# imironhead/ml_super_resolution

Measured on AMD Instinct MI355X. Metric: VDSR-20 training patches/sec (41x41, batch 256 per GPU); fwd HR megapixels/sec alongside, higher is better.
Workload: dtype f32; 1 GPU; BASELINE configs[2]: VDSR 20-layer 3x3x64 residual, RGB, batch 256x41x41 per GPU, fwd+bwd+TF-Adam, random-init weights; global_batch=256, patch=41, parallelism=dp1

## Files before the change

include/srx.h:

```cpp
#ifndef SRX_H_
#define SRX_H_

#include <stddef.h>
#include <stdint.h>

#ifdef __cplusplus
extern "C" {
#endif

typedef void* srx_stream_t;

typedef enum {
    SRX_OK = 0,
    SRX_ERR_BAD_ARG = -1,
    SRX_ERR_UNSUPPORTED = -2,
    SRX_ERR_WORKSPACE = -3,
    SRX_ERR_LAUNCH = -4,
    SRX_ERR_ALIGN = -5
} srx_status;

typedef enum { SRX_PAD_SAME = 0, SRX_PAD_VALID = 1 } srx_pad_mode;

typedef enum {
    SRX_ACT_NONE = 0,
    SRX_ACT_RELU = 1,
    SRX_ACT_TANH = 2,
    SRX_ACT_LRELU = 3,
    SRX_ACT_SIGMOID = 4
} srx_act;

typedef enum { SRX_OP_FWD = 0, SRX_OP_BWD_DATA = 1, SRX_OP_BWD_FILTER = 2 } srx_conv_op;

typedef enum { SRX_PRECISION_FP32 = 0, SRX_PRECISION_BF16X3 = 1 } srx_precision;

typedef struct {
    int32_t N, H, W, Cin, Cout, KH, KW;
    int32_t stride;
    int32_t pad_mode;
    int32_t act;
    int32_t post_add_relu;
    int32_t precision;
    int32_t subpixel_r;
} srx_conv_desc;

const char* srx_version(void);
const char* srx_last_error(void);

int srx_set_conv_path(int pipelined);

int srx_set_wgrad_path(int path);

int srx_conv2d_precision_supported(const srx_conv_desc* d, int op);

size_t srx_conv2d_workspace_bytes(const srx_conv_desc* d, int op);

int srx_conv2d_fwd(const srx_conv_desc* d, const float* x, const float* w, const float* bias,
                   const float* skip, float* y, void* ws, size_t ws_bytes, srx_stream_t stream);

int srx_conv2d_bwd_data(const srx_conv_desc* d, const float* dpre, const float* w,
                        const float* x_in, int in_act, float* dx_out, void* ws, size_t ws_bytes,
                        srx_stream_t stream);

int srx_conv2d_bwd_data_acc(const srx_conv_desc* d, const float* dpre, const float* w, const float* dx_acc,
                            float* dx_out, void* ws, size_t ws_bytes, srx_stream_t stream);

int srx_conv2d_bwd_filter(const srx_conv_desc* d, const float* x, const float* dpre, float* dw,
                          float* dbias, const float* w_for_decay, float wd_scale, void* ws,
                          size_t ws_bytes, srx_stream_t stream);

int srx_conv2d_bwd_filter_partials(const srx_conv_desc* d, const float* x, const float* dpre, void* ws,
                                   size_t ws_bytes, int* n_partials, srx_stream_t stream);
int srx_conv2d_bwd_filter_reduce(const srx_conv_desc* d, const void* ws, int n_partials, float* dw,
                                 float* dbias, const float* w_for_decay, float wd_scale,
                                 srx_stream_t stream);

int srx_act_bwd(const float* dy, const float* y, float* dpre, size_t numel, int act,
                srx_stream_t stream);

int srx_depth_to_space(const float* in, float* out, int N, int H, int W, int C, int r,
                       srx_stream_t stream);

int srx_stream_copy(const void* in, void* out, size_t bytes, srx_stream_t stream);

// ... 137 lines not shown
```

ml_super_resolution_amd/_lib.py:

```python
import ctypes
import os

_HERE = os.path.dirname(os.path.abspath(__file__))
LIB_PATH = os.path.join(_HERE, 'libsrx.so')

SRX_OK = 0
PAD_SAME, PAD_VALID = 0, 1
ACT_NONE, ACT_RELU, ACT_TANH, ACT_LRELU, ACT_SIGMOID = 0, 1, 2, 3, 4
OP_FWD, OP_BWD_DATA, OP_BWD_FILTER = 0, 1, 2
PRECISION_FP32, PRECISION_BF16X3 = 0, 1
PRECISION_BY_NAME = {'highest': PRECISION_FP32, 'high': PRECISION_BF16X3}

ACT_BY_NAME = {None: ACT_NONE, 'none': ACT_NONE, 'relu': ACT_RELU, 'tanh': ACT_TANH,
               'lrelu': ACT_LRELU, 'leaky_relu': ACT_LRELU, 'sigmoid': ACT_SIGMOID}
PAD_BY_NAME = {'same': PAD_SAME, 'valid': PAD_VALID}

EXPORTS = [
    'srx_version', 'srx_last_error', 'srx_set_conv_path', 'srx_set_wgrad_path', 'srx_conv2d_precision_supported', 'srx_conv2d_workspace_bytes', 'srx_conv2d_fwd',
    'srx_conv2d_bwd_data', 'srx_conv2d_bwd_filter', 'srx_conv2d_bwd_filter_partials', 'srx_conv2d_bwd_filter_reduce', 'srx_act_bwd', 'srx_depth_to_space',
    'srx_space_to_depth', 'srx_stream_copy', 'srx_mse_fwd_bwd', 'srx_l2_loss', 'srx_reduce_scratch_bytes',
    'srx_adam_tf_step', 'srx_adam_tf_step_dev', 'srx_momentum_clip_step', 'srx_rownorm_loss_fwd_bwd', 'srx_psnr', 'srx_ssim', 'srx_ssim_scratch_bytes', 'srx_saturate_u8', 'srx_affine', 'srx_u8_to_unit_float', 'srx_gaussian_blur', 'srx_resize_bilinear',
    'srx_upsample_nearest', 'srx_upsample_nearest_bwd', 'srx_add_relu_grad',
    'srx_conv2d_bwd_data_acc', 'srx_conv3x3_blocked', 'srx_conv3x3_blocked_bwd_filter_workspace_bytes', 'srx_conv3x3_blocked_bwd_filter',
    'srx_espcn_forward', 'srx_espcn_forward_keep', 'srx_debug_poison_lds', 'srx_srcnn_forward', 'srx_maxpool2x2', 'srx_maxpool2x2_bwd', 'srx_maxpool2x2_bwd_masked', 'srx_subsample2', 'srx_subsample2_bwd',
    'srx_channel_blocks_to_nhwc', 'srx_nhwc_to_channel_blocks', 'srx_channel_normalize', 'srx_channel_normalize_bwd',
    'srx_extract_patches16', 'srx_texture_gram', 'srx_texture_gram_bwd', 'srx_pil_resample_ksize', 'srx_pil_resample_coeffs', 'srx_resample_u8', 'srx_u8_to_pm1', 'srx_log_loss', 'srx_vgg_preprocess', 'srx_add_scaled', 'srx_resize_bicubic_tf', 'srx_column_sums', 'srx_gemm_workspace_bytes', 'srx_gemm',
]


class SrxError(RuntimeError):
    pass


class ConvDesc(ctypes.Structure):
    _fields_ = [(n, ctypes.c_int32) for n in
                ('N', 'H', 'W', 'Cin', 'Cout', 'KH', 'KW', 'stride', 'pad_mode', 'act',
                 'post_add_relu', 'precision', 'subpixel_r')]


class GemmDesc(ctypes.Structure):
    _fields_ = ([(n, ctypes.c_int32) for n in ('M', 'N', 'K', 'batch')] +
                [(n, ctypes.c_int64) for n in ('a_row_stride', 'a_col_stride', 'a_batch_stride', 'b_row_stride',
                                               'b_col_stride', 'b_batch_stride', 'c_row_stride', 'c_col_stride',
                                               'c_batch_stride')] +
                [('alpha', ctypes.c_float), ('act', ctypes.c_int32), ('accumulate', ctypes.c_int32)])


_lib = None


def lib():
    global _lib
    if _lib is not None:
        return _lib
    if not os.path.exists(LIB_PATH):
        raise SrxError('libsrx.so not found at %s -- build it with `make -C %s` (or '
                       '__graft_entry__.build()); there is no CPU fallback' %
                       (LIB_PATH, os.path.join(_HERE, 'csrc')))
    import torch
    L = ctypes.CDLL(LIB_PATH)
    vp, sz, i, f = ctypes.c_void_p, ctypes.c_size_t, ctypes.c_int, ctypes.c_float
    dp = ctypes.POINTER(ConvDesc)
    L.srx_version.restype = ctypes.c_char_p
    L.srx_last_error.restype = ctypes.c_char_p
    L.srx_set_conv_path.argtypes = [i]
    L.srx_set_wgrad_path.argtypes = [i]
    L.srx_conv2d_precision_supported.argtypes = [dp, i]
    L.srx_conv2d_workspace_bytes.argtypes = [dp, i]
    L.srx_conv2d_workspace_bytes.restype = sz
    L.srx_reduce_scratch_bytes.restype = sz
    L.srx_conv2d_fwd.argtypes = [dp, vp, vp, vp, vp, vp, vp, sz, vp]
    L.srx_conv2d_bwd_data.argtypes = [dp, vp, vp, vp, i, vp, vp, sz, vp]
    L.srx_conv2d_bwd_filter.argtypes = [dp, vp, vp, vp, vp, vp, f, vp, sz, vp]
    L.srx_conv2d_bwd_filter_partials.argtypes = [dp, vp, vp, vp, sz, ctypes.POINTER(ctypes.c_int), vp]
    L.srx_conv2d_bwd_filter_reduce.argtypes = [dp, vp, i, vp, vp, vp, f, vp]
    L.srx_act_bwd.argtypes = [vp, vp, vp, sz, i, vp]
    L.srx_depth_to_space.argtypes = [vp, vp, i, i, i, i, i, vp]
    L.srx_space_to_depth.argtypes = [vp, vp, i, i, i, i, i, vp]
    L.srx_stream_copy.argtypes = [vp, vp, sz, vp]
    L.srx_mse_fwd_bwd.argtypes = [vp, vp, sz, f, vp, i, vp, vp, vp]
    L.srx_l2_loss.argtypes = [vp, vp, sz, f, vp, i, vp, vp]
    L.srx_adam_tf_step.argtypes = [vp, vp, vp, vp, sz, f, f, f, f, ctypes.c_int64, f, vp]
    L.srx_adam_tf_step_dev.argtypes = [vp, vp, vp, vp, sz, vp, f, f, f, f, vp]
    L.srx_momentum_clip_step.argtypes = [vp, vp, vp, sz, f, f, f, f, vp]
    L.srx_rownorm_loss_fwd_bwd.argtypes = [vp, vp, sz, sz, vp, vp, vp, vp]
    L.srx_psnr.argtypes = [vp, vp, vp, i, sz, f, vp]
    L.srx_ssim.argtypes = [vp, vp, vp, i, i, i, i, f, vp, vp]
    L.srx_ssim_scratch_bytes.argtypes = [i]
    L.srx_ssim_scratch_bytes.restype = sz
    L.srx_saturate_u8.argtypes = [vp, vp, sz, vp]
    L.srx_affine.argtypes = [vp, vp, sz, f, f, vp]
    L.srx_u8_to_unit_float.argtypes = [vp, vp, sz, vp]
    L.srx_gaussian_blur.argtypes = [vp, vp, vp, i, i, i, i, f, vp]
    L.srx_resize_bilinear.argtypes = [vp, vp, i, i, i, i, i, i, vp]
    L.srx_upsample_nearest.argtypes = [vp, vp, i, i, i, i, i, vp]
    L.srx_upsample_nearest_bwd.argtypes = [vp, vp, i, i, i, i, i, vp]
    L.srx_add_relu_grad.argtypes = [vp, vp, vp, vp, sz, vp]
    L.srx_conv2d_bwd_data_acc.argtypes = [dp, vp, vp, vp, vp, vp, sz, vp]
    L.srx_espcn_forward.argtypes = [vp] * 8 + [i, i, i, i, vp]
# ... 41 lines not shown
```

ml_super_resolution_amd/csrc/conv_kernels.hip.h:

```cpp
#pragma once
#include <hip/hip_runtime.h>
#include <stdint.h>
#include <type_traits>

namespace srx {

typedef float f32x4 __attribute__((ext_vector_type(4)));

enum { ACT_NONE = 0, ACT_RELU = 1, ACT_TANH = 2, ACT_LRELU = 3, ACT_SIGMOID = 4 };

struct ConvArgs {
    const float* x;
    const float* w;
    const float* bias;
    const float* skip;
    const float* mask;
    float* y;
    int N, H, W, OH, OW, Cin, Cout;
    int pad_t, pad_l;
    int TH, TW, NTX, RS;
    int units_total;
    int act, post_relu, mask_act;
    float inv_rs;
    int stagger;
    int dbg;
    unsigned long long* trace;
    int buf_floats;
    int* tile_counter;
    int tiles_total, tiles_per_col;
    int lds_sched_slot;
    int stride;
    int d2s_r, d2s_rc;
};

struct WgradArgs {
    const float* x;
    const float* dpre;
    float* part;
    int part_stride;
    int N, H, W, OH, OW, Cin, Cout;
    int pad_t, pad_l;
    int TH, TW, NTX, RS;
    int units_total;
    float inv_rs;
    int stagger;
    int zero_slot;
    int stride;
    unsigned long long* trace;
};

template <int CINP>
struct Lds {
    static constexpr int PS = (CINP == 4) ? 4 : CINP + 4;
};

__device__ __forceinline__ float srx_tanhf(float x) {
    const float ax = fabsf(x);
    const float x2 = ax * ax;
    float p = fmaf(x2, -0.006274174898862839f, 0.021071631461381912f);
    p = fmaf(x2, p, -0.053852297365665436f);
    p = fmaf(x2, p, 0.13332585990428925f);
    p = fmaf(x2, p, -0.33333316445350647f);
    const float small = fmaf(x2 * ax, p, ax);
    const float e = __builtin_amdgcn_exp2f(ax * 2.8853900817779268f);
    const float big = fmaf(-2.0f, __builtin_amdgcn_rcpf(e + 1.0f), 1.0f);
    return copysignf(ax < 0.55f ? small : big, x);
}

typedef float f32x2 __attribute__((ext_vector_type(2)));
__device__ __forceinline__ f32x2 srx_tanhf2(f32x2 x) {
    const f32x2 ax = {fabsf(x[0]), fabsf(x[1])};
    const f32x2 x2 = ax * ax;
    f32x2 p = __builtin_elementwise_fma(x2, f32x2{-0.006274174898862839f, -0.006274174898862839f}, f32x2{0.021071631461381912f, 0.021071631461381912f});
    p = __builtin_elementwise_fma(x2, p, f32x2{-0.053852297365665436f, -0.053852297365665436f});
    p = __builtin_elementwise_fma(x2, p, f32x2{0.13332585990428925f, 0.13332585990428925f});
    p = __builtin_elementwise_fma(x2, p, f32x2{-0.33333316445350647f, -0.33333316445350647f});
    const f32x2 small = __builtin_elementwise_fma(x2 * ax, p, ax);
    const f32x2 t = ax * 2.8853900817779268f;
    f32x2 e = {__builtin_amdgcn_exp2f(t[0]), __builtin_amdgcn_exp2f(t[1])};
    e = e + 1.0f;
    const f32x2 r = {__builtin_amdgcn_rcpf(e[0]), __builtin_amdgcn_rcpf(e[1])};
// ... 908 lines not shown
                if (t < NST) {
                    if constexpr (Z) stg[t] = stage_fire_z(mv, mr, so, xrs, voff_lane);
                    else stg[t] = stage_fire(mk[t], so, xrs, voff_lane);
                }
                if (t >= NBLK / 2 && t < NBLK / 2 + NST) stage_next<PPP * PS * 4>(qc, SG.JP1, SG.rowfix_l);
            } else {
                if (t < NST) stage_next<PPP * CINP * 4>(qi, SG.JP1, SG.rowfix_g);
                if (t == A0) {
                    tcur += gs * TSTEP;
#pragma unroll
                    for (int i = 0; i < MAXG; ++i) lan[i] = *reinterpret_cast<const int*>(ldsb + tcur + i * TSTEP);
                }
            }
        }
#pragma unroll
        for (int i = 0; i < nfr; ++i) cg[i] = nxt[i];
    }
#pragma unroll
    for (int i = 0; i < MAXG; ++i) { cur[i] = cg[i]; la[i] = lan[i]; }
    if constexpr (G == 4)
        asm volatile("s_nop 15\n\ts_nop 7" : "+v"(acc[0]), "+v"(acc[1]), "+v"(acc[2]), "+v"(acc[3]));
    else
        asm volatile("s_nop 15\n\ts_nop 7" : "+v"(acc[0]), "+v"(acc[1]), "+v"(acc[2]));
#pragma unroll
    for (int i = 0; i < MAXG; ++i) {
        pd.acc[i] = (i < G) ? acc[i < G ? i : 0] : bias4;
        if (HASAUX) pd.aux[i] = (i < G) ? aux[i < G ? i : 0] : bias4;
    }
    pd.yrs = un.yrs; pd.m_first = m_first; pd.gs = gs;
    tt[1] += SRX_STAMP() - ts_m;
}

template <int KH, int KW, int CINP, int NCH, bool WT, int AUX, bool Z>
__device__ __forceinline__ void conv_pipe_body(const ConvArgs& a) {
    extern __shared__ __attribute__((aligned(16))) float lds[];
    constexpr int TAPS = KH * KW;
    constexpr int KSPT = CINP / 4;
    constexpr int NPART = 4 / NCH;
    constexpr int TPP = CINP / 4, PPP = 256 / TPP;
    constexpr int PS = Lds<CINP>::PS;
    constexpr int MAXG = 4;
    constexpr int TSTEP = 16 * PS * 4 * NPART;
    const int tid = threadIdx.x;
    const int lane = tid & 63;
    const int wave = __builtin_amdgcn_readfirstlane(tid >> 6);
    const int li = lane & 15, kq = lane >> 4;
    const int chunk = wave % NCH, part = wave / NCH;
    const int cout0 = chunk * 16;
    const int cb = cout0 + 4 * kq;
    const int c4 = tid % TPP, sp = tid / TPP;
    char* ldsb = reinterpret_cast<char*>(lds);

#ifdef SRX_TRACE
    const unsigned long long t_entry = __builtin_amdgcn_s_memtime(), rt_entry = __builtin_amdgcn_s_memrealtime();
#endif
    float wr[TAPS * KSPT];
    load_stationary_weights<TAPS, CINP, WT>(wr, a, cout0, li, kq);
    f32x4 bias4 = {0.f, 0.f, 0.f, 0.f};
    if (a.bias) {
#pragma unroll
        for (int e = 0; e < 4; ++e)
            if (cb + e < a.Cout) bias4[e] = a.bias[cb + e];
    }

    const long G_ = gridDim.x;
    const int u0 = (int)(((long)blockIdx.x * a.units_total) / G_);
    const int u1 = (int)(((long)(blockIdx.x + 1) * a.units_total) / G_);
    if (u0 >= u1) return;
    const int buf_bytes = a.buf_floats * 4;
    const int rows_full = a.TH + KH - 1;
    const int row_stride_b = a.RS * PS * 4;

    {
        const f32x4 z = {0.f, 0.f, 0.f, 0.f};
        for (int i = tid; !Z && i < (rows_full + 1) * a.pad_l * TPP; i += 256) {
            const int q = i / TPP, ch = i % TPP;
            const int r = q / a.pad_l, c = q % a.pad_l;
            const int off = ((r * a.RS + c) * PS + 4 * ch) * 4;
            if ((r * a.RS + c) * PS * 4 < buf_bytes) {
                *reinterpret_cast<f32x4*>(ldsb + off) = z;
                *reinterpret_cast<f32x4*>(ldsb + buf_bytes + off) = z;
            }
        }
        const int tw_ = Z ? a.TW : a.OW;
        const int n_sub_max = (a.TH * tw_ + 15) >> 4;
        for (int i = tid; i < n_sub_max * 64; i += 256) {
            const int m = i >> 6, L = i & 63;
            const int t = 16 * m + (L & 15);
            int addr = 0;
            if (t < a.TH * tw_) {
                const int orow = t / tw_, ocol = t - orow * tw_;
                addr = ((orow * a.RS + ocol) * PS + 4 * (L >> 4)) * 4;
            }
            const int where = ((16 * m + (L >> 2)) * PS + CINP + (L & 3)) * 4;
            *reinterpret_cast<int*>(ldsb + where) = addr;
            *reinterpret_cast<int*>(ldsb + buf_bytes + where) = buf_bytes + addr;
        }
    }
    const int voff_lane = tid * 16;
    const int wl_lane = (sp * PS + 4 * c4) * 4;
    int vst = (cb < a.Cout) ? (li * a.Cout + cb) * 4 : kOobOffset;
    const int tlane = (((lane >> 2) + 16 * part) * PS + CINP + (lane & 3)) * 4;
    StageGeo SG;
    const int JP = (a.RS + PPP - 1) / PPP;
    SG.JP1 = __builtin_amdgcn_readfirstlane(JP - 1);
    SG.rowfix_g = __builtin_amdgcn_readfirstlane((a.W - JP * PPP) * CINP * 4);
// ... 1660 lines not shown
```

ml_super_resolution_amd/csrc/launchers.h:

```cpp
#pragma once
#include "conv_kernels.hip.h"

namespace srx {

struct ConvKey {
    int kh, kw, cinp, nch;
    bool wt;
};

bool launch_conv_k3c64(const ConvKey& k, const ConvArgs& a, int grid, size_t lds, hipStream_t s, hipError_t* err);
bool launch_conv_k3c32(const ConvKey& k, const ConvArgs& a, int grid, size_t lds, hipStream_t s, hipError_t* err);
bool launch_conv_c4(const ConvKey& k, const ConvArgs& a, int grid, size_t lds, hipStream_t s, hipError_t* err);
bool launch_conv_misc(const ConvKey& k, const ConvArgs& a, int grid, size_t lds, hipStream_t s, hipError_t* err);
bool launch_pipe_k3c64(const ConvKey& k, const ConvArgs& a, int grid, size_t lds, hipStream_t s, hipError_t* err);
bool launch_pipe_other(const ConvKey& k, const ConvArgs& a, int grid, size_t lds, hipStream_t s, hipError_t* err);
bool launch_wgrad_narrow(const ConvKey& k, const WgradArgs& a, int grid, hipStream_t s, hipError_t* err);
bool launch_conv_narrow(const ConvKey& k, const ConvArgs& a, hipStream_t s, hipError_t* err);
bool launch_conv_1x1(const ConvKey& k, const ConvArgs& a, long min_pixels, hipStream_t s, hipError_t* err);
bool launch_conv_rows3x3(const ConvKey& k, const ConvArgs& a, long min_pixels, hipStream_t s, hipError_t* err);
bool launch_conv_pack3(const ConvKey& k, const ConvArgs& a, long min_pixels, hipStream_t s, hipError_t* err);
bool launch_conv_kwrows(const ConvKey& k, const ConvArgs& a, long min_pixels, hipStream_t s, hipError_t* err);
bool launch_pipe_strip(const ConvKey& k, const ConvArgs& a, int grid, size_t lds, hipStream_t s, hipError_t* err);
bool launch_conv_generic(const ConvKey& k, const ConvArgs& a, int grid, size_t lds, hipStream_t s, hipError_t* err);
bool launch_wgrad(const ConvKey& k, const WgradArgs& a, int grid, size_t lds, hipStream_t s, hipError_t* err);
bool launch_wgrad_generic(const ConvKey& k, const WgradArgs& a, int grid, size_t lds, hipStream_t s, hipError_t* err);
bool launch_wgrad_lin(const ConvKey& k, const WgradArgs& a, int grid, size_t lds, hipStream_t s, hipError_t* err);
bool launch_wgrad_lin_pack3(const ConvKey& k, const WgradArgs& a, int grid, size_t lds, hipStream_t s, hipError_t* err);
bool launch_wgrad_lin_strip(const ConvKey& k, const WgradArgs& a, int grid, size_t lds, hipStream_t s, hipError_t* err);
bool launch_wgrad_pipe(const ConvKey& k, const WgradArgs& a, int grid, size_t lds, hipStream_t s, hipError_t* err);
bool launch_wgrad_kwcols(const ConvKey& k, const WgradArgs& a, int max_partials, long min_pixels, int* n_partials, hipStream_t s, hipError_t* err);
bool launch_wgrad_1x1(const ConvKey& k, const WgradArgs& a, int max_partials, int* n_partials, hipStream_t s, hipError_t* err);
bool launch_wgrad_rows_full(const ConvKey& k, const WgradArgs& a, int grid, size_t lds, hipStream_t s, hipError_t* err);
bool launch_wgrad_rows_strip(const ConvKey& k, const WgradArgs& a, int grid, size_t lds, bool nt, hipStream_t s, hipError_t* err);
bool launch_wgrad_lin_pairs(const ConvKey& k, const WgradPairs& q, int grid, int pairs, bool strips, size_t lds, hipStream_t s, hipError_t* err);

hipError_t launch_reduce_partials(const float* part, int G, int stride, int wn, int cout, float* dw, float* dbias,
                                  const float* w, float wd, hipStream_t s);
hipError_t launch_reduce_partials_pairs(const float* part, int G, int stride, int wn, int cout, float* dw, float* dbias,
                                        int pairs, int cob, hipStream_t s);

template <typename K, typename A>
inline hipError_t launch_with_lds(K kernel, const A& a, int grid, size_t lds, hipStream_t s, int grid_y = 1) {
    static thread_local const void* configured[64];
    static thread_local int n_configured = 0;
    const void* fn = reinterpret_cast<const void*>(kernel);
    bool known = false;
    for (int i = 0; i < n_configured; ++i) known |= (configured[i] == fn);
    if (!known) {
        hipError_t e = hipFuncSetAttribute(fn, hipFuncAttributeMaxDynamicSharedMemorySize, 160 * 1024);
        if (e != hipSuccess) return e;
        if (n_configured < 64) configured[n_configured++] = fn;
    }
    hipLaunchKernelGGL(kernel, dim3(grid, grid_y), dim3(256), lds, s, a);
    return hipGetLastError();
}

#define SRX_CONV_CASE(KH, KW, CINP, NCH, WT, MINW)                                                        \
    if (k.kh == KH && k.kw == KW && k.cinp == CINP && k.nch == NCH && k.wt == WT) {                       \
        if (a.skip || a.mask)                                                                             \
            *err = launch_with_lds(conv_mfma_kernel<KH, KW, CINP, NCH, WT, MINW, true>, a, grid, lds, s); \
        else                                                                                              \
            *err = launch_with_lds(conv_mfma_kernel<KH, KW, CINP, NCH, WT, MINW, false>, a, grid, lds, s);\
        return true;                                                                                      \
    }
#define SRX_PIPE_CASE_FWD(KH, KW, CINP, NCH)                                                              \
    if (k.kh == KH && k.kw == KW && k.cinp == CINP && k.nch == NCH && !k.wt) {                            \
        if (a.skip)                                                                                       \
            *err = launch_with_lds(conv_pipe_kernel<KH, KW, CINP, NCH, false, 2>, a, grid, lds, s);       \
        else                                                                                              \
            *err = launch_with_lds(conv_pipe_kernel<KH, KW, CINP, NCH, false, 0>, a, grid, lds, s);       \
        return true;                                                                                      \
    }
#define SRX_PIPE_CASE_DGRAD(KH, KW, CINP, NCH)                                                            \
    if (k.kh == KH && k.kw == KW && k.cinp == CINP && k.nch == NCH && k.wt) {                             \
        if (a.mask)                                                                                       \
            *err = launch_with_lds(conv_pipe_kernel<KH, KW, CINP, NCH, true, 1>, a, grid, lds, s);        \
        else                                                                                              \
            *err = launch_with_lds(conv_pipe_kernel<KH, KW, CINP, NCH, true, 0>, a, grid, lds, s);        \
        return true;                                                                                      \
    }
#define SRX_PIPE_STRIP_CASE(KH, KW, CINP, NCH)                                                            \
    if (k.kh == KH && k.kw == KW && k.cinp == CINP && k.nch == NCH && !k.wt) {                            \
        if (a.skip)                                                                                       \
            *err = launch_with_lds(conv_pipe_strip_kernel<KH, KW, CINP, NCH, false, 2>, a, grid, lds, s); \
        else                                                                                              \
            *err = launch_with_lds(conv_pipe_strip_kernel<KH, KW, CINP, NCH, false, 0>, a, grid, lds, s); \
// ... 45 lines not shown
```

ml_super_resolution_amd/csrc/srx_api.hip:

```cpp
#include <math.h>
#include <stdarg.h>
#include <atomic>
#include <stdio.h>
#include <stdlib.h>
#include <string.h>

#include "../../include/srx.h"
#include "elementwise.h"
#include "launchers.h"
#include "bf16x3.h"

using namespace srx;

namespace {

thread_local char g_err[512] = "";

struct Knobs {
    int pipe_default, min_full_th, small_rule, th, grid, narrow, dyn, stagger, wgrad_lin, wgrad_pipe, wgrad_pipe_strip, wgrad_rows_full, wgrad_1x1, wgrad_pack3, wgrad_nt, kwrows_min_pixels, big_route_min_pixels, strip_d2s, conv_1x1_min_pixels, pack3_dgrad;
    int subpixel_chunk_kb, subpixel_db, subpixel_grid, subpixel_depth, subpixel_throttle, subpixel_even;
    unsigned long long* trace;
    int dbg;
};
int env_int(const char* name, int dflt) { const char* e = getenv(name); return e ? atoi(e) : dflt; }
Knobs read_knobs() {
    Knobs k;
    k.pipe_default = env_int("SRX_PIPE", 1);
    k.min_full_th = env_int("SRX_MIN_FULL_TH", 3);
    k.small_rule = env_int("SRX_SMALL_RULE", 1);
    k.th = env_int("SRX_TH", -1);
    k.grid = env_int("SRX_GRID", -1);
    k.narrow = env_int("SRX_NARROW", 1);
    k.dyn = env_int("SRX_DYN", 0);
    k.stagger = env_int("SRX_STAGGER", -1);
    k.wgrad_lin = env_int("SRX_WGRAD_LIN", 1);
    k.wgrad_pipe = env_int("SRX_WGRAD_PIPE", 1);
    k.wgrad_pipe_strip = env_int("SRX_WGRAD_PIPE_STRIP", 1);
    k.kwrows_min_pixels = env_int("SRX_KWROWS_MIN_PIXELS", 4096);
    k.big_route_min_pixels = env_int("SRX_BIG_ROUTE_MIN_PIXELS", 60000);
    k.conv_1x1_min_pixels = env_int("SRX_CONV_1X1_MIN_PIXELS", 100000);
    k.pack3_dgrad = env_int("SRX_PACK3_DGRAD", 1);
    k.strip_d2s = env_int("SRX_STRIP_D2S", 1);
    k.wgrad_rows_full = env_int("SRX_WGRAD_ROWS_FULL", 1);
    k.wgrad_1x1 = env_int("SRX_WGRAD_1X1", 1);
    k.wgrad_pack3 = env_int("SRX_WGRAD_PACK3", 1);
    k.wgrad_nt = env_int("SRX_WGRAD_NT", 1);
    k.subpixel_chunk_kb = env_int("SRX_SUBPIXEL_CHUNK_KB", 24);
    k.subpixel_db = env_int("SRX_SUBPIXEL_DB", 1);
    k.subpixel_grid = env_int("SRX_SUBPIXEL_GRID", 0);
    k.subpixel_depth = env_int("SRX_SUBPIXEL_DEPTH", 0);
    k.subpixel_throttle = env_int("SRX_SUBPIXEL_THROTTLE", -1);
    k.subpixel_even = env_int("SRX_SUBPIXEL_EVEN", 1);
    k.trace = nullptr;
    k.dbg = 0;
#ifdef SRX_TRACE
    { const char* tp = getenv("SRX_TRACE_PTR"); k.trace = tp ? (unsigned long long*)strtoull(tp, nullptr, 0) : nullptr; }
    k.dbg = env_int("SRX_DBG", 0);
#endif
    return k;
}
const Knobs& knobs() { static const Knobs k = read_knobs(); return k; }

std::atomic<int> g_use_pipe{-1};
int use_pipe() { const int v = g_use_pipe.load(std::memory_order_relaxed); return v < 0 ? knobs().pipe_default : v; }
std::atomic<int> g_wgrad_path{-1};
int wgrad_path_default() { return !knobs().wgrad_lin ? 0 : ((knobs().wgrad_pipe || knobs().wgrad_pipe_strip) ? 2 : 1); }
int wgrad_path() { const int v = g_wgrad_path.load(std::memory_order_relaxed); return v < 0 ? wgrad_path_default() : v; }

int cu_count() {
    static std::atomic<int> cached[64];
    int dev = 0;
    if (hipGetDevice(&dev) != hipSuccess || dev < 0 || dev >= 64) { (void)hipGetLastError(); return 256; }
    int n = cached[dev].load(std::memory_order_relaxed);
    if (n > 0) return n;
    if (hipDeviceGetAttribute(&n, hipDeviceAttributeMultiprocessorCount, dev) != hipSuccess || n <= 0) {
        (void)hipGetLastError();
        n = 256;
    }
    if (n > 256) n = 256;
    cached[dev].store(n, std::memory_order_relaxed);
    return n;
}

int fail(int code, const char* fmt, ...) {
    va_list ap;
    va_start(ap, fmt);
    vsnprintf(g_err, sizeof(g_err), fmt, ap);
    va_end(ap);
    return code;
}
}
namespace srx {
int set_error(int code, const char* fmt, ...) {
    va_list ap;
    va_start(ap, fmt);
    vsnprintf(g_err, sizeof(g_err), fmt, ap);
// ... 292 lines not shown
    }
    bool hit = launch_conv_k3c64(k, a, p.grid, p.lds_bytes, s, &err) ||
               launch_conv_k3c32(k, a, p.grid, p.lds_bytes, s, &err) ||
               launch_conv_c4(k, a, p.grid, p.lds_bytes, s, &err) ||
               launch_conv_misc(k, a, p.grid, p.lds_bytes, s, &err) ||
               launch_conv_generic(k, a, p.grid, p.lds_bytes, s, &err);
    if (!hit)
        return fail(SRX_ERR_UNSUPPORTED, "no kernel instance for %dx%d, Cin<=%d, Cout chunks %d, %s", p.KH, p.KW,
                    p.cinp, p.nch, wt ? "dgrad" : "fwd");
    if (err != hipSuccess) return fail(SRX_ERR_LAUNCH, "conv launch failed: %s", hipGetErrorString(err));
    return SRX_OK;
}

int stagger_sleeps(const Plan& p) {
    const int env = knobs().stagger;
    if (env >= 0) return env;
    if (p.grid < max_grid()) return 0;
    const long tiles_per_wg = (long)p.units_total / ((long)p.grid * p.TH);
    return tiles_per_wg >= 2 ? 4 : 0;
}

void fill_conv_args(ConvArgs* a, const Plan& p, int N, int H, int W, int in_c, int out_c) {
    a->N = N; a->H = H; a->W = W; a->OH = p.OH; a->OW = p.OW; a->Cin = in_c; a->Cout = out_c;
    a->pad_t = p.pad_t; a->pad_l = p.pad_l;
    a->TH = p.TH; a->TW = p.TW; a->NTX = p.NTX; a->RS = p.RS;
    a->units_total = p.units_total;
    a->inv_rs = 1.0f / (float)p.RS;
    a->stride = 1;
    a->stagger = stagger_sleeps(p);
    a->dbg = knobs().dbg;
    a->trace = knobs().trace;
}

}

extern "C" {

const char* srx_version(void) { return "srx 0.1 (gfx950, fp32 MFMA 16x16x4)"; }
const char* srx_last_error(void) { return g_err; }
int srx_set_conv_path(int pipelined) {
    const int old = g_use_pipe.exchange(pipelined ? 1 : 0, std::memory_order_relaxed);
    return old < 0 ? knobs().pipe_default : old;
}
int srx_set_wgrad_path(int path) {
    const int old = g_wgrad_path.exchange(path < 0 ? -1 : (path > 2 ? 2 : path), std::memory_order_relaxed);
    return old < 0 ? wgrad_path_default() : old;
}
size_t srx_reduce_scratch_bytes(void) { return (size_t)kReduceBlocks * sizeof(float); }

int srx_conv2d_precision_supported(const srx_conv_desc* d, int op) {
    if (check_desc(d) != SRX_OK) return 0;
    if (op != SRX_OP_FWD && op != SRX_OP_BWD_DATA && op != SRX_OP_BWD_FILTER) { fail(SRX_ERR_BAD_ARG, "bad op %d", op); return 0; }
    if (d->precision == SRX_PRECISION_FP32) return 1;
    return bf16x3_supported(d, op) == SRX_OK ? 1 : 0;
}

size_t srx_conv2d_workspace_bytes(const srx_conv_desc* d, int op) {
    if (check_desc(d) != SRX_OK) return 0;
    if (d->precision == SRX_PRECISION_BF16X3) {
        if (bf16x3_supported(d, op) != SRX_OK) return 0;
        if (op != SRX_OP_BWD_FILTER) return 256;
        Bf3Plan bp;
        bf16x3_plan(d->N, d->H, d->W, max_grid(), true, &bp);
        return (size_t)bp.grid * part_stride(d) * sizeof(float);
    }
    if (op != SRX_OP_BWD_FILTER) return 256;
    int pt, pl, OH, OW;
    geometry(d, &pt, &pl, &OH, &OW);
    Plan p;
// ... 506 lines not shown
```

ml_super_resolution_amd/engine.py:

```python
import math
import os

import torch

from . import ops


class LayerSpec(object):

    def __init__(self, ksize, cin, cout, padding='same', act=None, scope=None):
        self.kh, self.kw = (ksize, ksize) if isinstance(ksize, int) else ksize
        self.cin, self.cout = cin, cout
        self.padding = padding.lower()
        self.act = act
        self.scope = scope

    @property
    def kernel_shape(self):
        return (self.kh, self.kw, self.cin, self.cout)

    def out_hw(self, h, w):
        if self.padding == 'same':
            return h, w
        return h - self.kh + 1, w - self.kw + 1
# ... 90 lines not shown

    def set_params(self, pairs):
        for i, (k, b) in enumerate(pairs):
            self.kernel(i).copy_(torch.as_tensor(k, dtype=torch.float32).to(self.device))
            self.bias(i).copy_(torch.as_tensor(b, dtype=torch.float32).to(self.device))

    def _buf(self, key, shape):
        t = self._bufs.get(key)
        if t is None or tuple(t.shape) != tuple(shape):
            if t is not None:
                self._step_graphs.clear()
            t = torch.empty(shape, dtype=torch.float32, device=self.device)
            self._bufs[key] = t
        return t

    def _shapes(self, x_shape):
        n, h, w, _ = x_shape
        shapes = []
        for s in self.specs:
            h, w = s.out_hw(h, w)
            shapes.append((n, h, w, s.cout))
        return shapes

    def forward(self, x, keep=True):
        shapes = self._shapes(x.shape)
        if keep and self.forward_keep_hook is not None:
            outs = [self._buf(('act', i), shapes[i]) for i in range(len(self.specs))]
            if self.forward_keep_hook(x, outs):
                self._acts = self.acts = [x] + outs
                return outs[-1]
        acts = [x]
        t = x
        last = len(self.specs) - 1
        for i, s in enumerate(self.specs):
            skip = x if (self.residual and i == last) else None
            if keep:
                out = self._buf(('act', i), shapes[i])
            else:
                out = self._buf(('tmp', i & 1, s.cout), shapes[i])
            t = ops.conv2d_fwd(t, self.kernel(i), self.bias(i), s.padding, s.act, skip=skip, out=out,
                               precision=self.layer_precision[i])
            acts.append(t)
        self._acts = acts if keep else None
        self.acts = acts
        return t

    def loss_and_backward(self, target, numel_global=None):
        if self._acts is None:
            raise RuntimeError('forward(keep=True) must run before loss_and_backward')
        acts = self._acts
        y = acts[-1]
        last = len(self.specs) - 1
        inv = 1.0 / (y.numel() if numel_global is None else numel_global)
        if self.loss_kind == 'rownorm':
            row_len = y.shape[1] * y.shape[2]
            dy = ops.rownorm_loss_fwd_bwd(y, target, row_len, self.loss, dpred=self._buf(('dy', 0), y.shape),
                                          norms=self._buf(('rownorms',), (y.numel() // row_len,)))
        else:
            dy = self._buf(('dy', 0), y.shape)
            ops.mse_fwd_bwd(y, target, self.loss, inv_numel=inv, accumulate=False, dpred=dy)
        if self.weight_decay:
            self.add_regulariser_loss()
        if self.specs[last].act is not None:
            dpre = ops.act_bwd(dy, y, self.specs[last].act, out=self._buf(('dpre_last',), y.shape))
        else:
            dpre = dy
        prec = self.layer_precision
        need = max(ops.bwd_filter_workspace_bytes(acts[i].shape, s.kernel_shape, s.padding, precision=prec[i])
                   for i, s in enumerate(self.specs))
        if self._ws is None or self._ws.numel() * 4 < need:
            self._step_graphs.clear()
            self._ws = torch.empty((need + 3) // 4, dtype=torch.float32, device=self.device)
            self._ws2 = None
        main = torch.cuda.current_stream(self.device) if self.device.type == 'cuda' else None
        two = self.overlap_wgrad and main is not None
        if two and self._side is None:
            self._side = torch.cuda.Stream(device=self.device)
        red = self.overlap_reduce and main is not None and not two
        if red:
            if self._side is None:
                self._side = torch.cuda.Stream(device=self.device)
            if self._ws2 is None or self._ws2.numel() != self._ws.numel():
                self._ws2 = torch.empty_like(self._ws)
        ws_free = [None, None]
        read_done = {}
        for i in range(last, -1, -1):
            s = self.specs[i]
            if red:
                k = i & 1
                ws = self._ws if k == 0 else self._ws2
                if ws_free[k] is not None:
                    main.wait_event(ws_free[k])
                n_part = ops.conv2d_bwd_filter_partials(acts[i], dpre, s.kernel_shape, s.padding, ws, precision=prec[i])
                ready = torch.cuda.Event()
                ready.record(main)
                with torch.cuda.stream(self._side):
                    self._side.wait_event(ready)
                    ops.conv2d_bwd_filter_reduce(acts[i].shape, s.kernel_shape, s.padding, ws, n_part,
                                                 self.kernel(i, self.grads), self.bias(i, self.grads),
                                                 w_for_decay=self.kernel(i) if self.weight_decay else None,
                                                 wd_scale=self.weight_decay, precision=prec[i])
                    ws_free[k] = torch.cuda.Event()
                    ws_free[k].record(self._side)
            elif two:
                ready = torch.cuda.Event()
                ready.record(main)
                with torch.cuda.stream(self._side):
                    self._side.wait_event(ready)
                    ops.conv2d_bwd_filter(acts[i], dpre, s.kernel_shape, s.padding,
                                          w_for_decay=self.kernel(i) if self.weight_decay else None,
                                          wd_scale=self.weight_decay, dw=self.kernel(i, self.grads),
                                          dbias=self.bias(i, self.grads), workspace=self._ws, precision=prec[i])
                    done = torch.cuda.Event()
                    done.record(self._side)
                read_done[dpre.data_ptr()] = done
            else:
                ops.conv2d_bwd_filter(acts[i], dpre, s.kernel_shape, s.padding,
                                      w_for_decay=self.kernel(i) if self.weight_decay else None,
                                      wd_scale=self.weight_decay, dw=self.kernel(i, self.grads),
                                      dbias=self.bias(i, self.grads), workspace=self._ws, precision=prec[i])
# ... 205 lines not shown
```

ml_super_resolution_amd/ops.py:

```python
import ctypes
import os

import torch

from . import _lib
from ._lib import ACT_BY_NAME, PAD_BY_NAME, ConvDesc, check
from ._lib import lib as _load_lib

_POISON_LDS = os.environ.get('SRX_POISON_LDS', '0') == '1'


def lib():
    L = _load_lib()
    if _POISON_LDS and torch.cuda.is_available():
        L.srx_debug_poison_lds(_stream())
    return L



def _stream():
    return ctypes.c_void_p(torch.cuda.current_stream().cuda_stream)


def _ptr(t):
# ... 61 lines not shown
        _scratch[key] = torch.empty(lib().srx_reduce_scratch_bytes() // 4, dtype=torch.float32, device=device)
    return _scratch[key]


def conv2d_fwd(x, w, bias=None, padding='same', act=None, skip=None, post_add_relu=False, out=None, subpixel_r=0, stride=1,
               precision='highest'):
    for t, n in ((x, 'x'), (w, 'w'), (bias, 'bias'), (skip, 'skip')):
        _chk(t, n)
    d = conv_desc(x.shape, w.shape, padding, act, post_add_relu, subpixel_r, stride, precision)
    shape = out_shape(d)
    if subpixel_r > 1:
        r = int(subpixel_r)
        if shape[3] % (r * r):
            raise ValueError('subpixel_r %d: %d output channels are not a multiple of r*r' % (r, shape[3]))
        shape = (shape[0], shape[1] * r, shape[2] * r, shape[3] // (r * r))
    if out is not None and tuple(out.shape) != tuple(shape):
        raise ValueError('out has shape %s, expected %s' % (tuple(out.shape), tuple(shape)))
    y = out if out is not None else torch.empty(shape, dtype=torch.float32, device=x.device)
    ws = sched_workspace(x.device)
    check(lib().srx_conv2d_fwd(ctypes.byref(d), _ptr(x), _ptr(w), _ptr(bias), _ptr(skip), _ptr(y),
                               ctypes.c_void_p(ws.data_ptr()), 256, _stream()), 'srx_conv2d_fwd')
    return y


def conv2d_bwd_data(dpre, w, x_shape, padding='same', x_in=None, in_act=None, out=None, precision='highest'):
    for t, n in ((dpre, 'dpre'), (w, 'w'), (x_in, 'x_in')):
        _chk(t, n)
    d = conv_desc(x_shape, w.shape, padding, precision=precision)
    dx = out if out is not None else torch.empty(tuple(x_shape), dtype=torch.float32, device=dpre.device)
    ws = sched_workspace(dpre.device)
    check(lib().srx_conv2d_bwd_data(ctypes.byref(d), _ptr(dpre), _ptr(w), _ptr(x_in), ACT_BY_NAME[in_act],
                                    _ptr(dx), ctypes.c_void_p(ws.data_ptr()), 256, _stream()), 'srx_conv2d_bwd_data')
    return dx


def bwd_filter_workspace_bytes(x_shape, w_shape, padding='same', stride=1, precision='highest'):
    d = conv_desc(x_shape, w_shape, padding, stride=stride, precision=precision)
    return lib().srx_conv2d_workspace_bytes(ctypes.byref(d), _lib.OP_BWD_FILTER)


def conv2d_bwd_filter(x, dpre, w_shape, padding='same', w_for_decay=None, wd_scale=0.0, dw=None, dbias=None,
                      want_dbias=True, workspace=None, stride=1, precision='highest'):
    for t, n in ((x, 'x'), (dpre, 'dpre'), (w_for_decay, 'w_for_decay')):
        _chk(t, n)
    d = conv_desc(x.shape, w_shape, padding, stride=stride, precision=precision)
    if tuple(dpre.shape) != tuple(out_shape(d)):
        raise ValueError('dpre has shape %s, the layer output is %s' % (tuple(dpre.shape), tuple(out_shape(d))))
    if dw is None:
        dw = torch.empty(tuple(w_shape), dtype=torch.float32, device=x.device)
    if dbias is None and want_dbias:
        dbias = torch.empty((w_shape[3],), dtype=torch.float32, device=x.device)
    need = lib().srx_conv2d_workspace_bytes(ctypes.byref(d), _lib.OP_BWD_FILTER)
    if workspace is None:
        workspace = torch.empty((need + 3) // 4, dtype=torch.float32, device=x.device)
    check(lib().srx_conv2d_bwd_filter(ctypes.byref(d), _ptr(x), _ptr(dpre), _ptr(dw), _ptr(dbias),
                                      _ptr(w_for_decay), float(wd_scale), _ptr(workspace),
                                      workspace.numel() * 4, _stream()), 'srx_conv2d_bwd_filter')
    return dw, dbias


def conv2d_bwd_filter_partials(x, dpre, w_shape, padding, workspace, precision='highest'):
    _chk(x, 'x'); _chk(dpre, 'dpre'); _chk(workspace, 'workspace')
    d = conv_desc(x.shape, w_shape, padding, precision=precision)
    n = ctypes.c_int(0)
    check(lib().srx_conv2d_bwd_filter_partials(ctypes.byref(d), _ptr(x), _ptr(dpre), _ptr(workspace), workspace.numel() * 4,
                                               ctypes.byref(n), _stream()), 'srx_conv2d_bwd_filter_partials')
# ... 532 lines not shown
```

Before: 18650 patches/s.

## Chain consecutive 3x3 64-channel conv layers into one persistent kernel launch

Adds a chain kernel that runs several identical 3x3 64->64 conv layers, forward or data-gradient, in a single launch. Each workgroup owns whole images, so layers only need a workgroup-level barrier between them, and the LDS zero-padding setup runs once. The engine groups eligible VDSR middle layers into these chains in the forward pass, and in backward when the two-stream and reduce wgrad paths are off. The aim is to remove per-layer launch gaps and keep each image's activations warm in cache across layers. In exchange, grid size is limited to divisors of the batch, and a chained backward gives up the overlapped side-stream weight-gradient reduction.

```diff
diff --git a/include/srx.h b/include/srx.h
--- a/include/srx.h
+++ b/include/srx.h
@@ -49,6 +49,13 @@
 int srx_set_conv_path(int pipelined);
 
 int srx_set_wgrad_path(int path);
+
+int srx_conv_chain(const srx_conv_desc* d, int op, int in_act, int layers, const float* const* x, const float* const* w,
+                   const float* const* bias, const float* const* aux, float* const* y, srx_stream_t stream);
+
+int srx_conv_chain_supported(const srx_conv_desc* d, int op, int in_act);
+
+int srx_set_chain(int on);
 
 int srx_conv2d_precision_supported(const srx_conv_desc* d, int op);
 
diff --git a/ml_super_resolution_amd/_lib.py b/ml_super_resolution_amd/_lib.py
--- a/ml_super_resolution_amd/_lib.py
+++ b/ml_super_resolution_amd/_lib.py
@@ -16,7 +16,7 @@
 PAD_BY_NAME = {'same': PAD_SAME, 'valid': PAD_VALID}
 
 EXPORTS = [
-    'srx_version', 'srx_last_error', 'srx_set_conv_path', 'srx_set_wgrad_path', 'srx_conv2d_precision_supported', 'srx_conv2d_workspace_bytes', 'srx_conv2d_fwd',
+    'srx_version', 'srx_last_error', 'srx_set_conv_path', 'srx_set_wgrad_path', 'srx_set_chain', 'srx_conv_chain', 'srx_conv_chain_supported', 'srx_conv2d_precision_supported', 'srx_conv2d_workspace_bytes', 'srx_conv2d_fwd',
     'srx_conv2d_bwd_data', 'srx_conv2d_bwd_filter', 'srx_conv2d_bwd_filter_partials', 'srx_conv2d_bwd_filter_reduce', 'srx_act_bwd', 'srx_depth_to_space',
     'srx_space_to_depth', 'srx_stream_copy', 'srx_mse_fwd_bwd', 'srx_l2_loss', 'srx_reduce_scratch_bytes',
     'srx_adam_tf_step', 'srx_adam_tf_step_dev', 'srx_momentum_clip_step', 'srx_rownorm_loss_fwd_bwd', 'srx_psnr', 'srx_ssim', 'srx_ssim_scratch_bytes', 'srx_saturate_u8', 'srx_affine', 'srx_u8_to_unit_float', 'srx_gaussian_blur', 'srx_resize_bilinear',
@@ -65,6 +65,9 @@
     L.srx_last_error.restype = ctypes.c_char_p
     L.srx_set_conv_path.argtypes = [i]
     L.srx_set_wgrad_path.argtypes = [i]
+    L.srx_set_chain.argtypes = [i]
+    L.srx_conv_chain_supported.argtypes = [dp, i, i]
+    L.srx_conv_chain.argtypes = [dp, i, i, i, vp, vp, vp, vp, vp, vp]
     L.srx_conv2d_precision_supported.argtypes = [dp, i]
     L.srx_conv2d_workspace_bytes.argtypes = [dp, i]
     L.srx_conv2d_workspace_bytes.restype = sz
diff --git a/ml_super_resolution_amd/csrc/conv_chain.hip b/ml_super_resolution_amd/csrc/conv_chain.hip
--- /dev/null
+++ b/ml_super_resolution_amd/csrc/conv_chain.hip
@@ -0,0 +1,27 @@
+#include "launchers.h"
+namespace srx {
+
+template <bool WT, int AUX>
+__global__ __launch_bounds__(256, 1) void conv_chain_kernel(const ConvArgs a, const ChainPtrs c) {
+    for (int l = 0; l < c.L; ++l) {
+        ConvArgs al = a;
+        al.x = c.x[l]; al.w = c.w[l]; al.bias = c.bias[l]; al.y = c.y[l];
+        if (WT) al.mask = c.aux[l];
+        else al.skip = c.aux[l];
+        asm volatile("" : "+s"(al.N), "+s"(al.H), "+s"(al.W), "+s"(al.OH), "+s"(al.OW), "+s"(al.Cin), "+s"(al.Cout));
+        asm volatile("" : "+s"(al.pad_t), "+s"(al.pad_l), "+s"(al.TH), "+s"(al.TW), "+s"(al.NTX), "+s"(al.RS));
+        asm volatile("" : "+s"(al.units_total), "+s"(al.act), "+s"(al.post_relu), "+s"(al.mask_act), "+s"(al.buf_floats));
+        conv_pipe_body<3, 3, 64, 4, WT, AUX, false>(al, l == 0);
+        asm volatile("s_waitcnt vmcnt(0)" ::: "memory");
+        __builtin_amdgcn_fence(__ATOMIC_RELEASE, "workgroup");
+        __builtin_amdgcn_s_barrier();
+        __builtin_amdgcn_fence(__ATOMIC_ACQUIRE, "workgroup");
+    }
+}
+
+hipError_t launch_conv_chain(bool wt, bool aux, const ConvArgs& a, const ChainPtrs& c, int grid, size_t lds, hipStream_t s) {
+    if (!wt) return aux ? hipErrorInvalidValue : launch_chain_with_lds(conv_chain_kernel<false, 0>, a, c, grid, lds, s);
+    return aux ? launch_chain_with_lds(conv_chain_kernel<true, 1>, a, c, grid, lds, s)
+               : launch_chain_with_lds(conv_chain_kernel<true, 0>, a, c, grid, lds, s);
+}
+}
diff --git a/ml_super_resolution_amd/csrc/conv_kernels.hip.h b/ml_super_resolution_amd/csrc/conv_kernels.hip.h
--- a/ml_super_resolution_amd/csrc/conv_kernels.hip.h
+++ b/ml_super_resolution_amd/csrc/conv_kernels.hip.h
@@ -47,6 +47,16 @@
     int zero_slot;
     int stride;
     unsigned long long* trace;
+};
+
+constexpr int kChainMax = 32;
+struct ChainPtrs {
+    const float* x[kChainMax];
+    const float* w[kChainMax];
+    const float* bias[kChainMax];
+    const float* aux[kChainMax];
+    float* y[kChainMax];
+    int L;
 };
 
 template <int CINP>
@@ -1021,7 +1031,7 @@
 }
 
 template <int KH, int KW, int CINP, int NCH, bool WT, int AUX, bool Z>
-__device__ __forceinline__ void conv_pipe_body(const ConvArgs& a) {
+__device__ __forceinline__ void conv_pipe_body(const ConvArgs& a, bool lds_setup = true) {
     extern __shared__ __attribute__((aligned(16))) float lds[];
     constexpr int TAPS = KH * KW;
     constexpr int KSPT = CINP / 4;
@@ -1060,7 +1070,7 @@
     const int rows_full = a.TH + KH - 1;
     const int row_stride_b = a.RS * PS * 4;
 
-    {
+    if (lds_setup) {
         const f32x4 z = {0.f, 0.f, 0.f, 0.f};
         for (int i = tid; !Z && i < (rows_full + 1) * a.pad_l * TPP; i += 256) {
             const int q = i / TPP, ch = i % TPP;
diff --git a/ml_super_resolution_amd/csrc/launchers.h b/ml_super_resolution_amd/csrc/launchers.h
--- a/ml_super_resolution_amd/csrc/launchers.h
+++ b/ml_super_resolution_amd/csrc/launchers.h
@@ -34,6 +34,8 @@
 bool launch_wgrad_rows_strip(const ConvKey& k, const WgradArgs& a, int grid, size_t lds, bool nt, hipStream_t s, hipError_t* err);
 bool launch_wgrad_lin_pairs(const ConvKey& k, const WgradPairs& q, int grid, int pairs, bool strips, size_t lds, hipStream_t s, hipError_t* err);
 
+__attribute__((weak)) hipError_t launch_conv_chain(bool wt, bool aux, const ConvArgs& a, const ChainPtrs& c, int grid, size_t lds, hipStream_t s);
+
 hipError_t launch_reduce_partials(const float* part, int G, int stride, int wn, int cout, float* dw, float* dbias,
                                   const float* w, float wd, hipStream_t s);
 hipError_t launch_reduce_partials_pairs(const float* part, int G, int stride, int wn, int cout, float* dw, float* dbias,
@@ -52,6 +54,22 @@
         if (n_configured < 64) configured[n_configured++] = fn;
     }
     hipLaunchKernelGGL(kernel, dim3(grid, grid_y), dim3(256), lds, s, a);
+    return hipGetLastError();
+}
+
+template <typename K>
+inline hipError_t launch_chain_with_lds(K kernel, const ConvArgs& a, const ChainPtrs& c, int grid, size_t lds, hipStream_t s) {
+    static thread_local const void* configured[8];
+    static thread_local int n_configured = 0;
+    const void* fn = reinterpret_cast<const void*>(kernel);
+    bool known = false;
+    for (int i = 0; i < n_configured; ++i) known |= (configured[i] == fn);
+    if (!known) {
+        hipError_t e = hipFuncSetAttribute(fn, hipFuncAttributeMaxDynamicSharedMemorySize, 160 * 1024);
+        if (e != hipSuccess) return e;
+        if (n_configured < 8) configured[n_configured++] = fn;
+    }
+    hipLaunchKernelGGL(kernel, dim3(grid), dim3(256), lds, s, a, c);
     return hipGetLastError();
 }
 
diff --git a/ml_super_resolution_amd/csrc/srx_api.hip b/ml_super_resolution_amd/csrc/srx_api.hip
--- a/ml_super_resolution_amd/csrc/srx_api.hip
+++ b/ml_super_resolution_amd/csrc/srx_api.hip
@@ -19,6 +19,7 @@
 struct Knobs {
     int pipe_default, min_full_th, small_rule, th, grid, narrow, dyn, stagger, wgrad_lin, wgrad_pipe, wgrad_pipe_strip, wgrad_rows_full, wgrad_1x1, wgrad_pack3, wgrad_nt, kwrows_min_pixels, big_route_min_pixels, strip_d2s, conv_1x1_min_pixels, pack3_dgrad;
     int subpixel_chunk_kb, subpixel_db, subpixel_grid, subpixel_depth, subpixel_throttle, subpixel_even;
+    int chain;
     unsigned long long* trace;
     int dbg;
 };
@@ -51,6 +52,7 @@
     k.subpixel_depth = env_int("SRX_SUBPIXEL_DEPTH", 0);
     k.subpixel_throttle = env_int("SRX_SUBPIXEL_THROTTLE", -1);
     k.subpixel_even = env_int("SRX_SUBPIXEL_EVEN", 1);
+    k.chain = env_int("SRX_CHAIN", 1);
     k.trace = nullptr;
     k.dbg = 0;
 #ifdef SRX_TRACE
@@ -62,6 +64,8 @@
 const Knobs& knobs() { static const Knobs k = read_knobs(); return k; }
 
 std::atomic<int> g_use_pipe{-1};
+std::atomic<int> g_chain{-1};
+int use_chain() { const int v = g_chain.load(std::memory_order_relaxed); return v < 0 ? (knobs().chain ? 1 : 0) : v; }
 int use_pipe() { const int v = g_use_pipe.load(std::memory_order_relaxed); return v < 0 ? knobs().pipe_default : v; }
 std::atomic<int> g_wgrad_path{-1};
 int wgrad_path_default() { return !knobs().wgrad_lin ? 0 : ((knobs().wgrad_pipe || knobs().wgrad_pipe_strip) ? 2 : 1); }
@@ -420,9 +424,87 @@
     a->trace = knobs().trace;
 }
 
+int chain_plan(const srx_conv_desc* d, int op, int in_act, Plan* p, ConvArgs* a, int* grid) {
+    int rc = check_desc(d);
+    if (rc) return rc;
+    if (op != SRX_OP_FWD && op != SRX_OP_BWD_DATA) return fail(SRX_ERR_BAD_ARG, "chain: op %d (forward or data gradient)", op);
+    if (!use_chain()) return fail(SRX_ERR_UNSUPPORTED, "chain: switched off (srx_set_chain / SRX_CHAIN)");
+    if (!use_pipe()) return fail(SRX_ERR_UNSUPPORTED, "chain: conv path 0");
+    if (!launch_conv_chain) return fail(SRX_ERR_UNSUPPORTED, "chain: this build has no chain kernels");
+    if (d->precision != SRX_PRECISION_FP32) return fail(SRX_ERR_UNSUPPORTED, "chain: precision %d (exact fp32 only)", d->precision);
+    if (d->KH != 3 || d->KW != 3 || d->Cin != 64 || d->Cout != 64 || d->stride != 1 || d->pad_mode != SRX_PAD_SAME)
+        return fail(SRX_ERR_UNSUPPORTED, "chain: only 3x3 64->64 stride-1 SAME layers");
+    if (d->subpixel_r > 1 || d->post_add_relu) return fail(SRX_ERR_UNSUPPORTED, "chain: no sub-pixel store or post-add activation");
+    if (op == SRX_OP_FWD && d->act != SRX_ACT_NONE && d->act != SRX_ACT_RELU)
+        return fail(SRX_ERR_UNSUPPORTED, "chain: forward activation %d (none / ReLU)", d->act);
+    if (op == SRX_OP_BWD_DATA && in_act != SRX_ACT_NONE && in_act != SRX_ACT_RELU)
+        return fail(SRX_ERR_UNSUPPORTED, "chain: in_act %d (none / ReLU)", in_act);
+    int pt, pl, OH, OW;
+    geometry(d, &pt, &pl, &OH, &OW);
+    rc = (op == SRX_OP_FWD) ? make_plan(d->N, d->H, d->W, OH, OW, d->Cin, d->Cout, 3, 3, pt, pl, p, true)
+                            : make_plan(d->N, OH, OW, d->H, d->W, d->Cout, d->Cin, 3, 3, 2 - pt, 2 - pl, p);
+    if (rc) return rc;
+    memset(a, 0, sizeof(*a));
+    if (op == SRX_OP_FWD) fill_conv_args(a, *p, d->N, d->H, d->W, d->Cin, d->Cout);
+    else fill_conv_args(a, *p, d->N, OH, OW, d->Cout, d->Cin);
+    a->act = (op == SRX_OP_FWD) ? d->act : SRX_ACT_NONE;
+    a->post_relu = 0;
+    a->mask_act = (op == SRX_OP_FWD) ? 0 : in_act;
+    a->trace = nullptr;
+    const int ppp = 256 / (p->cinp / 4);
+    const bool pipe_ok = p->cinp == 64 && p->nch == 4 && p->NTX == 1 && p->RS >= ppp && p->RS == a->W + a->pad_l && 16 <= a->OW &&
+                         (long)a->H * a->W * a->Cin * 4 < (1L << 31) - 64 && (long)a->OH * a->OW * a->Cout * 4 < (1L << 31) - 64;
+    if (!pipe_ok) return fail(SRX_ERR_UNSUPPORTED, "chain: the shape is not on the full-width pipelined route (column strips?)");
+    *grid = p->grid < pipe_grid() ? p->grid : pipe_grid();
+    if (d->N % *grid) return fail(SRX_ERR_UNSUPPORTED, "chain: N %d is not a multiple of the grid %d (a workgroup would split an image)", d->N, *grid);
+    a->buf_floats = (int)(p->lds_bytes / 4);
+    return SRX_OK;
+}
+
 }
 
 extern "C" {
+
+int srx_set_chain(int on) {
+    const int old = g_chain.exchange(on < 0 ? -1 : (on ? 1 : 0), std::memory_order_relaxed);
+    return old < 0 ? (knobs().chain ? 1 : 0) : old;
+}
+
+int srx_conv_chain_supported(const srx_conv_desc* d, int op, int in_act) {
+    Plan p;
+    ConvArgs a;
+    int grid;
+    return chain_plan(d, op, in_act, &p, &a, &grid) == SRX_OK ? 1 : 0;
+}
+
+int srx_conv_chain(const srx_conv_desc* d, int op, int in_act, int layers, const float* const* x, const float* const* w,
+                   const float* const* bias, const float* const* aux, float* const* y, srx_stream_t stream) {
+    if (layers < 1 || layers > kChainMax) return fail(SRX_ERR_BAD_ARG, "chain: %d layers (1..%d)", layers, kChainMax);
+    if (!x || !w || !y) return fail(SRX_ERR_BAD_ARG, "null pointer array");
+    Plan p;
+    ConvArgs a;
+    int grid;
+    int rc = chain_plan(d, op, in_act, &p, &a, &grid);
+    if (rc) return rc;
+    const bool wt = op == SRX_OP_BWD_DATA;
+    const bool masked = wt && in_act == SRX_ACT_RELU;
+    ChainPtrs c;
+    memset(&c, 0, sizeof(c));
+    c.L = layers;
+    for (int l = 0; l < layers; ++l) {
+        const float* m = aux ? aux[l] : nullptr;
+        if (!x[l] || !w[l] || !y[l]) return fail(SRX_ERR_BAD_ARG, "chain: null tensor pointer in layer %d", l);
+        if (!wt && m) return fail(SRX_ERR_UNSUPPORTED, "chain: the forward skip operand is not implemented");
+        if (masked != (m != nullptr)) return fail(SRX_ERR_BAD_ARG, "chain: layer %d: a mask goes with in_act ReLU, and only with it", l);
+        if (!aligned16(x[l]) || !aligned16(w[l]) || !aligned16(y[l]) || (m && !aligned16(m)) || (bias && bias[l] && (reinterpret_cast<uintptr_t>(bias[l]) & 3)))
+            return fail(SRX_ERR_ALIGN, "tensor base pointers must be 16-byte aligned");
+        if (y[l] == x[l] || (m && y[l] == m)) return fail(SRX_ERR_BAD_ARG, "chain: layer %d writes its own operand", l);
+        c.x[l] = x[l]; c.w[l] = w[l]; c.bias[l] = (bias && !wt) ? bias[l] : nullptr; c.aux[l] = m; c.y[l] = y[l];
+    }
+    const hipError_t err = launch_conv_chain(wt, masked, a, c, grid, 2 * p.lds_bytes, (hipStream_t)stream);
+    if (err != hipSuccess) return fail(SRX_ERR_LAUNCH, "chain launch failed: %s", hipGetErrorString(err));
+    return SRX_OK;
+}
 
 const char* srx_version(void) { return "srx 0.1 (gfx950, fp32 MFMA 16x16x4)"; }
 const char* srx_last_error(void) { return g_err; }
diff --git a/ml_super_resolution_amd/engine.py b/ml_super_resolution_amd/engine.py
--- a/ml_super_resolution_amd/engine.py
+++ b/ml_super_resolution_amd/engine.py
@@ -146,18 +146,64 @@
         acts = [x]
         t = x
         last = len(self.specs) - 1
-        for i, s in enumerate(self.specs):
+
+        def out_buf(i):
+            if keep:
+                return self._buf(('act', i), shapes[i])
+            return self._buf(('tmp', i & 1, self.specs[i].cout), shapes[i])
+
+        i = 0
+        while i <= last:
+            s = self.specs[i]
+            j = self._chain_end(i, [x.shape] + shapes, ops._lib.OP_FWD)
+            if j > i + 1:
+                outs = [out_buf(k) for k in range(i, j)]
+                xs = [t] + outs[:-1]
+                t = ops.conv2d_fwd_chain(xs, [self.kernel(k) for k in range(i, j)], [self.bias(k) for k in range(i, j)], outs,
+                                         s.padding, s.act)
+                acts.extend(outs)
+                i = j
+                continue
             skip = x if (self.residual and i == last) else None
-            if keep:
-                out = self._buf(('act', i), shapes[i])
-            else:
-                out = self._buf(('tmp', i & 1, s.cout), shapes[i])
-            t = ops.conv2d_fwd(t, self.kernel(i), self.bias(i), s.padding, s.act, skip=skip, out=out,
+            t = ops.conv2d_fwd(t, self.kernel(i), self.bias(i), s.padding, s.act, skip=skip, out=out_buf(i),
                                precision=self.layer_precision[i])
             acts.append(t)
+            i += 1
         self._acts = acts if keep else None
         self.acts = acts
         return t
+
+    def _chain_ok(self, i, in_shape, op):
+        s = self.specs[i]
+        if self.layer_precision[i] != 'highest' or s.kh != 3 or s.kw != 3 or s.cin != 64 or s.cout != 64 or s.act not in (None, 'relu'):
+            return False
+        if op == ops._lib.OP_FWD:
+            if self.residual and i == len(self.specs) - 1:
+                return False
+            return ops.chain_supported(in_shape, s.kernel_shape, op, s.padding, s.act)
+        if i == 0 or self.specs[i - 1].act not in (None, 'relu'):
+            return False
+        return ops.chain_supported(in_shape, s.kernel_shape, op, s.padding, in_act=self.specs[i - 1].act)
+
+    def _chain_end(self, i, in_shapes, op):
+        s = self.specs[i]
+        j = i
+        while (j < len(self.specs) and j - i < 32 and self.specs[j].padding == s.padding and self.specs[j].act == s.act and
+               tuple(in_shapes[j]) == tuple(in_shapes[i]) and self._chain_ok(j, in_shapes[j], op)):
+            j += 1
+        return j
+
+    def _dgrad_chain(self, acts):
+        last = len(self.specs) - 1
+        for hi in range(last - 1, 0, -1):
+            s = self.specs[hi]
+            lo = hi
+            while (lo >= 1 and hi - lo < 32 and self.specs[lo].padding == s.padding and self.specs[lo - 1].act == self.specs[hi - 1].act and
+                   tuple(acts[lo].shape) == tuple(acts[hi].shape) and self._chain_ok(lo, acts[lo].shape, ops._lib.OP_BWD_DATA)):
+                lo -= 1
+            if hi - lo >= 2:
+                return lo + 1, hi
+        return None
 
     def loss_and_backward(self, target, numel_global=None):
         if self._acts is None:
@@ -198,8 +244,26 @@
                 self._ws2 = torch.empty_like(self._ws)
         ws_free = [None, None]
         read_done = {}
+        chain = None if (two or red) else self._dgrad_chain(acts)
         for i in range(last, -1, -1):
             s = self.specs[i]
+            if chain is not None and chain[0] <= i <= chain[1]:
+                lo, hi = chain
+                if i == hi:
+                    outs = [self._buf(('dpre_chain', k - 1), acts[k].shape) for k in range(hi, lo - 1, -1)]
+                    ops.conv2d_bwd_data_chain([dpre] + outs[:-1], [self.kernel(k) for k in range(hi, lo - 1, -1)],
+                                              [acts[k] for k in range(hi, lo - 1, -1)], outs, acts[hi].shape, s.padding,
+                                              in_act=self.specs[hi - 1].act)
+                    dpres = {hi: dpre}
+                    for k in range(hi, lo - 1, -1):
+                        dpres[k - 1] = outs[hi - k]
+                ops.conv2d_bwd_filter(acts[i], dpres[i], s.kernel_shape, s.padding,
+                                      w_for_decay=self.kernel(i) if self.weight_decay else None,
+                                      wd_scale=self.weight_decay, dw=self.kernel(i, self.grads),
+                                      dbias=self.bias(i, self.grads), workspace=self._ws, precision=prec[i])
+                if i == lo:
+                    dpre = dpres[lo - 1]
+                continue
             if red:
                 k = i & 1
                 ws = self._ws if k == 0 else self._ws2
diff --git a/ml_super_resolution_amd/ops.py b/ml_super_resolution_amd/ops.py
--- a/ml_super_resolution_amd/ops.py
+++ b/ml_super_resolution_amd/ops.py
@@ -117,6 +117,47 @@
     check(lib().srx_conv2d_bwd_data(ctypes.byref(d), _ptr(dpre), _ptr(w), _ptr(x_in), ACT_BY_NAME[in_act],
                                     _ptr(dx), ctypes.c_void_p(ws.data_ptr()), 256, _stream()), 'srx_conv2d_bwd_data')
     return dx
+
+
+def chain_supported(x_shape, w_shape, op=_lib.OP_FWD, padding='same', act=None, in_act=None, precision='highest'):
+    d = conv_desc(x_shape, w_shape, padding, act, precision=precision)
+    return lib().srx_conv_chain_supported(ctypes.byref(d), int(op), ACT_BY_NAME[in_act]) == 1
+
+
+def _ptr_array(ts):
+    return (ctypes.c_void_p * len(ts))(*[None if t is None else t.data_ptr() for t in ts])
+
+
+def conv2d_fwd_chain(xs, ws, biases, outs, padding='same', act=None):
+    for l in range(len(xs)):
+        _chk(xs[l], 'x'); _chk(ws[l], 'w'); _chk(biases[l], 'bias'); _chk(outs[l], 'out')
+    d = conv_desc(xs[0].shape, ws[0].shape, padding, act)
+    shape = out_shape(d)
+    for l in range(len(xs)):
+        if tuple(xs[l].shape) != tuple(xs[0].shape) or tuple(ws[l].shape) != tuple(ws[0].shape) or tuple(outs[l].shape) != shape:
+            raise ValueError('conv2d_fwd_chain: layer %d does not have the shape of layer 0' % l)
+    check(lib().srx_conv_chain(ctypes.byref(d), _lib.OP_FWD, _lib.ACT_NONE, len(xs), _ptr_array(xs), _ptr_array(ws), _ptr_array(biases),
+                               None, _ptr_array(outs), _stream()), 'srx_conv_chain')
+    return outs[-1]
+
+
+def conv2d_bwd_data_chain(dpres, ws, x_ins, outs, x_shape, padding='same', in_act=None):
+    masks = x_ins if (x_ins is not None and in_act is not None) else None
+    for l in range(len(dpres)):
+        _chk(dpres[l], 'dpre'); _chk(ws[l], 'w'); _chk(outs[l], 'out')
+        if masks is not None:
+            _chk(masks[l], 'x_in')
+        if tuple(outs[l].shape) != tuple(x_shape) or tuple(ws[l].shape) != tuple(ws[0].shape) or tuple(dpres[l].shape) != tuple(dpres[0].shape):
+            raise ValueError('conv2d_bwd_data_chain: layer %d does not have the shape of layer 0' % l)
+    d = conv_desc(x_shape, ws[0].shape, padding)
+    check(lib().srx_conv_chain(ctypes.byref(d), _lib.OP_BWD_DATA, ACT_BY_NAME[in_act] if masks is not None else _lib.ACT_NONE, len(dpres),
+                               _ptr_array(dpres), _ptr_array(ws), None, None if masks is None else _ptr_array(masks),
+                               _ptr_array(outs), _stream()), 'srx_conv_chain')
+    return outs[-1]
+
+
+def set_chain(on):
+    return lib().srx_set_chain(int(on))
 
 
 def bwd_filter_workspace_bytes(x_shape, w_shape, padding='same', stride=1, precision='highest'):
```

Measured after the change: 18930 patches/s, median of 6. +1.5%, better.
